# mit-han-lab/litepose

Hardware: AMD Instinct MI355X
Metric: images/sec end-to-end (backbone+deconv+AE-group), LitePose-XS@256 b64 (higher is better)
Workload: dtype f32

## Files before the change

### litepose_amd/csrc/ae_api.cpp

```cpp
#include <hip/hip_runtime.h>

#include <cstring>
#include <string>

#include "../../include/litepose_amd.h"
#include "kernels.h"

extern "C" void lp_set_error_(const char* msg);

namespace {
int fail(int code, const char* msg) {
    lp_set_error_(msg);
    return code;
}
size_t align256(size_t v) { return (v + 255) / 256 * 256; }

int to_params(const lp_parse_params* p, lp::ParseParams& q) {
    if (!p) return fail(LP_ERR_INVALID_ARG, "null params");
    if (p->num_joints < 1 || p->num_joints > 32) return fail(LP_ERR_UNSUPPORTED, "num_joints must be 1..32");
    if (p->max_num_people < 1 || p->max_num_people > 32)
        return fail(LP_ERR_UNSUPPORTED, "max_num_people must be 1..32");
    if (!(p->detection_threshold >= 0.0)) return fail(LP_ERR_INVALID_ARG, "detection_threshold must be >= 0");
    if (p->nms_kernel < 1 || (p->nms_kernel & 1) == 0) return fail(LP_ERR_INVALID_ARG, "nms_kernel must be odd");
    q.J = p->num_joints;
// ... 116 lines not shown
    lp::ScaleTable t;
    for (int s = 0; s < lp::MAX_SCALES; ++s) t.s[s] = {nullptr, 0, 0};
    for (int s = 0; s < S; ++s) {
        if (!scales[s].mid) return fail(LP_ERR_INVALID_ARG, "null mid");
        if (scales[s].h1 < 1 || scales[s].w1 < 1 || scales[s].h1 > 32767 || scales[s].w1 > 32767)
            return fail(LP_ERR_INVALID_ARG, "stage-1 sizes must be 1..32767");
        t.s[s] = {scales[s].mid, scales[s].h1, scales[s].w1};
    }
    if (!project2image && (Hf != scales[0].h1 || Wf != scales[0].w1))
        return fail(LP_ERR_INVALID_ARG, "without project2image (Hf, Wf) is the first scale's stage-1 size");
    if (T == 2 && ((uintptr_t)d_tag & 7)) return fail(LP_ERR_INVALID_ARG, "d_tag must be 8-byte aligned");
    if ((int64_t)N * 4 * J > 0x7fffffff) return fail(LP_ERR_UNSUPPORTED, "N * J too large");
    lp::launch_tta_merge_scales(t, S, first_unit, N, J, T, project2image ? 1 : 0, Hf, Wf, d_det, d_tag,
                                (hipStream_t)stream);
    if (hipGetLastError() != hipSuccess) return fail(LP_ERR_HIP, "tta_merge_scales launch failed");
    return LP_OK;
}

int lp_maps_accumulate(float* d_acc, const float* d_src, int64_t count, void* stream) {
    if (!d_acc || !d_src) return fail(LP_ERR_INVALID_ARG, "null argument");
    if (count < 0) return fail(LP_ERR_INVALID_ARG, "negative count");
    if (((uintptr_t)d_acc | (uintptr_t)d_src) & 15) return fail(LP_ERR_INVALID_ARG, "maps must be 16-byte aligned");
    if (count == 0) return LP_OK;
    lp::launch_maps_accumulate(d_acc, d_src, (long)count, (hipStream_t)stream);
    if (hipGetLastError() != hipSuccess) return fail(LP_ERR_HIP, "accumulate launch failed");
    return LP_OK;
}

int lp_peaks_topk(const float* d_det, const float* d_tag, int N, int J, int H, int W, int T,
                  const lp_parse_params* p, float* d_val_k, int32_t* d_ind_k, float* d_tag_k, void* stream) {
    lp::ParseParams q;
    int rc = to_params(p, q);
    if (rc) return rc;
    if (!d_det || !d_tag || !d_val_k || !d_ind_k || !d_tag_k) return fail(LP_ERR_INVALID_ARG, "null argument");
    if (J != q.J || T < 1 || T > 4 || N < 1 || H < 1 || W < 1) return fail(LP_ERR_INVALID_ARG, "bad dims");
    (void)lp::launch_peaks_topk(d_det, d_tag, N, J, H, W, T, q, d_val_k, d_ind_k, d_tag_k, (hipStream_t)stream);
    if (hipGetLastError() != hipSuccess) return fail(LP_ERR_HIP, "peaks_topk launch failed");
    return LP_OK;
}

int lp_group(const float* d_val_k, const int32_t* d_ind_k, const float* d_tag_k, int N, int W, int T,
             const lp_parse_params* p, int pcap, float* d_ans, int32_t* d_count, void* stream) {
    lp::ParseParams q;
    int rc = to_params(p, q);
    if (rc) return rc;
    if (!d_val_k || !d_ind_k || !d_tag_k || !d_ans || !d_count) return fail(LP_ERR_INVALID_ARG, "null argument");
    if (T < 1 || T > 4 || pcap < 1 || N < 1) return fail(LP_ERR_INVALID_ARG, "bad dims");
    lp::launch_group(d_val_k, d_ind_k, d_tag_k, N, W, T, q, pcap, d_ans, d_count, (hipStream_t)stream);
    if (hipGetLastError() != hipSuccess) return fail(LP_ERR_HIP, "group launch failed");
    return LP_OK;
}

size_t lp_refine_workspace_bytes(int N, int pcap) {
    return align256((size_t)N * pcap * 4 * sizeof(float)) + align256((size_t)N * pcap * sizeof(unsigned));
}

int lp_adjust_refine(const float* d_det, const float* d_tag, int N, int J, int H, int W, int T, int pcap,
                     int do_adjust, int do_refine, float* d_ans, const int32_t* d_count, float* d_scores,
                     void* ws, size_t ws_bytes, void* stream) {
    if (!d_det || !d_tag || !d_ans || !d_count || !d_scores || !ws)
        return fail(LP_ERR_INVALID_ARG, "null argument");
    if (T < 1 || T > 2) return fail(LP_ERR_UNSUPPORTED, "refine supports tag dimension 1 or 2");
    if (J < 1 || J > 32 || pcap < 1 || pcap > 1024) return fail(LP_ERR_UNSUPPORTED, "J 1..32, pcap 1..1024");
    if (ws_bytes < lp_refine_workspace_bytes(N, pcap)) return fail(LP_ERR_WORKSPACE, "refine workspace too small");
    float* prev = (float*)ws;
    unsigned* miss = (unsigned*)((char*)ws + align256((size_t)N * pcap * 4 * sizeof(float)));
    hipStream_t s = (hipStream_t)stream;
    lp::launch_adjust_scores(d_det, d_tag, N, J, H, W, T, pcap, do_adjust, d_ans, d_count, d_scores, prev,
                             miss, s);
    if (do_refine) lp::launch_refine(d_det, d_tag, N, J, H, W, T, pcap, d_ans, d_count, prev, miss, s);
    if (hipGetLastError() != hipSuccess) return fail(LP_ERR_HIP, "adjust/refine launch failed");
    return LP_OK;
}

size_t lp_parse_workspace_bytes(int N, int J, int M, int T, int pcap) {
    const size_t e = (size_t)N * J * M;
    return align256(e * sizeof(float)) + align256(e * sizeof(int)) + align256(e * T * sizeof(float)) +
           lp_refine_workspace_bytes(N, pcap);
}

int lp_parse(const float* d_det, const float* d_tag, int N, int J, int H, int W, int T,
             const lp_parse_params* p, int pcap, int do_adjust, int do_refine, float* d_ans,
             int32_t* d_count, float* d_scores, void* ws, size_t ws_bytes, void* stream) {
    if (!p || !ws) return fail(LP_ERR_INVALID_ARG, "null argument");
    const int M = p->max_num_people;
    if (ws_bytes < lp_parse_workspace_bytes(N, J, M, T, pcap))
        return fail(LP_ERR_WORKSPACE, "parse workspace too small");
    const size_t e = (size_t)N * J * M;
    char* c = (char*)ws;
    float* val_k = (float*)c;            c += align256(e * sizeof(float));
    int* ind_k = (int*)c;                c += align256(e * sizeof(int));
    float* tag_k = (float*)c;            c += align256(e * T * sizeof(float));
    int rc = lp_peaks_topk(d_det, d_tag, N, J, H, W, T, p, val_k, ind_k, tag_k, stream);
    if (rc) return rc;
    rc = lp_group(val_k, ind_k, tag_k, N, W, T, p, pcap, d_ans, d_count, stream);
    if (rc) return rc;
    return lp_adjust_refine(d_det, d_tag, N, J, H, W, T, pcap, do_adjust, do_refine, d_ans, d_count,
                            d_scores, c, lp_refine_workspace_bytes(N, pcap), stream);
}

int lp_parse_mid(const float* d_mid, int N, int J, int h1, int w1, int T, const lp_parse_params* p, int pcap,
                 int do_adjust, int do_refine, float* d_ans, int32_t* d_count, float* d_scores, void* ws,
                 size_t ws_bytes, void* stream) {
    lp::ParseParams q;
    int rc = to_params(p, q);
    if (rc) return rc;
    if (!d_mid || !d_ans || !d_count || !d_scores || !ws) return fail(LP_ERR_INVALID_ARG, "null argument");
    if (J != q.J || T < 1 || T > 2 || N < 1 || h1 < 1 || w1 < 1) return fail(LP_ERR_INVALID_ARG, "bad dims");
    if (pcap < 1 || pcap > 1024) return fail(LP_ERR_UNSUPPORTED, "pcap 1..1024");
    const int M = q.M;
    if (ws_bytes < lp_parse_workspace_bytes(N, J, M, T, pcap))
        return fail(LP_ERR_WORKSPACE, "parse workspace too small");
    const size_t e = (size_t)N * J * M;
    char* c = (char*)ws;
    float* val_k = (float*)c;            c += align256(e * sizeof(float));
    int* ind_k = (int*)c;                c += align256(e * sizeof(int));
    float* tag_k = (float*)c;            c += align256(e * T * sizeof(float));
    float* prev = (float*)c;
    unsigned* miss = (unsigned*)(c + align256((size_t)N * pcap * 4 * sizeof(float)));
    hipStream_t s = (hipStream_t)stream;
    if (!lp::launch_peaks_topk_walk(d_mid, N, J, h1, w1, T, q, val_k, ind_k, tag_k, s) &&
        !lp::launch_peaks_topk_mid(d_mid, N, J, h1, w1, T, q, val_k, ind_k, tag_k, s))
        return fail(LP_ERR_UNSUPPORTED, "lp_parse_mid: NMS radius 1..3, max_num_people <= 64, width <= 1024, "
                                        "TAG_PER_JOINT only (use lp_tta_project + lp_parse)");
    lp::launch_group(val_k, ind_k, tag_k, N, 2 * w1, T, q, pcap, d_ans, d_count, s);
    lp::launch_adjust_scores_mid(d_mid, N, J, h1, w1, T, pcap, do_adjust, d_ans, d_count, d_scores, prev, miss, s);
    if (do_refine && !lp::launch_refine_dm(nullptr, d_mid, N, J, h1, w1, T, pcap, d_ans, d_count, prev, miss, s))
        lp::launch_refine_mid(d_mid, N, J, h1, w1, T, pcap, d_ans, d_count, prev, miss, s);
    if (hipGetLastError() != hipSuccess) return fail(LP_ERR_HIP, "parse_mid launch failed");
    return LP_OK;
}

int lp_parse_dm(const float* d_det, const float* d_mid, int N, int J, int h1, int w1, int T,
                const lp_parse_params* p, int pcap, int do_adjust, int do_refine, float* d_ans, int32_t* d_count,
                float* d_scores, void* ws, size_t ws_bytes, void* stream) {
    lp::ParseParams q;
    int rc = to_params(p, q);
    if (rc) return rc;
    if (!d_det || !d_mid || !d_ans || !d_count || !d_scores || !ws) return fail(LP_ERR_INVALID_ARG, "null argument");
    if (J != q.J || T < 1 || T > 2 || N < 1 || h1 < 1 || w1 < 1) return fail(LP_ERR_INVALID_ARG, "bad dims");
    if (pcap < 1 || pcap > 1024) return fail(LP_ERR_UNSUPPORTED, "pcap 1..1024");
    const int M = q.M, H = 2 * h1, W = 2 * w1;
    if (ws_bytes < lp_parse_workspace_bytes(N, J, M, T, pcap))
        return fail(LP_ERR_WORKSPACE, "parse workspace too small");
    const size_t e = (size_t)N * J * M;
    char* c = (char*)ws;
    float* val_k = (float*)c;            c += align256(e * sizeof(float));
    int* ind_k = (int*)c;                c += align256(e * sizeof(int));
    float* tag_k = (float*)c;            c += align256(e * T * sizeof(float));
    float* prev = (float*)c;
    unsigned* miss = (unsigned*)(c + align256((size_t)N * pcap * 4 * sizeof(float)));
    hipStream_t s = (hipStream_t)stream;
    if (w1 > 1024 || !lp::launch_peaks_topk(d_det, nullptr, N, J, H, W, T, q, val_k, ind_k, tag_k, s, d_mid))
        return fail(LP_ERR_UNSUPPORTED, "lp_parse_dm: NMS radius 1..3, max_num_people <= 64, W % 4 == 0, w1 <= 1024, "
                                        "TAG_PER_JOINT only (use lp_tta_project + lp_parse)");
    lp::launch_group(val_k, ind_k, tag_k, N, W, T, q, pcap, d_ans, d_count, s);
    lp::launch_adjust_scores_mid(d_mid, N, J, h1, w1, T, pcap, do_adjust, d_ans, d_count, d_scores, prev, miss, s);
    if (do_refine && !lp::launch_refine_dm(d_det, d_mid, N, J, h1, w1, T, pcap, d_ans, d_count, prev, miss, s))
        return fail(LP_ERR_UNSUPPORTED, "lp_parse_dm: refine not supported for this shape (its gate and the one above "
                                        "have diverged); use lp_tta_project + lp_parse");
    if (hipGetLastError() != hipSuccess) return fail(LP_ERR_HIP, "parse_dm launch failed");
    return LP_OK;
}

int lp_warp_invert(const double* h_trans, double* h_minv) {
    if (!h_trans || !h_minv) return fail(LP_ERR_INVALID_ARG, "null argument");
    double M[6] = {h_trans[0], h_trans[1], h_trans[2], h_trans[3], h_trans[4], h_trans[5]};
    double D = M[0] * M[4] - M[1] * M[3];
    D = D != 0.0 ? 1.0 / D : 0.0;
    const double A11 = M[4] * D, A22 = M[0] * D;
    M[0] = A11; M[1] *= -D;
    M[3] *= -D; M[4] = A22;
    const double b1 = -M[0] * M[2] - M[1] * M[5];
    const double b2 = -M[3] * M[2] - M[4] * M[5];
    M[2] = b1; M[5] = b2;
    for (int i = 0; i < 6; ++i) h_minv[i] = M[i];
    return LP_OK;
}

int lp_preprocess(const uint8_t* d_image, int H, int W, const double* h_trans, int Hd, int Wd,
                  const float* h_mean, const float* h_std, uint8_t* d_resized_u8, float* d_tensor,
                  void* stream) {
    return lp_preprocess_batch(d_image, 1, H, W, h_trans, Hd, Wd, h_mean, h_std, d_resized_u8, d_tensor, stream);
}

int lp_preprocess_batch(const uint8_t* d_image, int N, int H, int W, const double* h_trans, int Hd, int Wd,
                        const float* h_mean, const float* h_std, uint8_t* d_resized_u8, float* d_tensor,
                        void* stream) {
    if (!d_image || !h_trans || !h_mean || !h_std) return fail(LP_ERR_INVALID_ARG, "null argument");
    if (N < 1 || N > 65535) return fail(LP_ERR_INVALID_ARG, "N must be 1..65535");
    if (!d_resized_u8 && !d_tensor) return fail(LP_ERR_INVALID_ARG, "no output requested");
    if (H < 1 || W < 1 || Hd < 1 || Wd < 1 || H > 32767 || W > 32767 || Hd > 32767 || Wd > 32767)
        return fail(LP_ERR_INVALID_ARG, "image sizes must be 1..32767");
    for (int c = 0; c < 3; ++c)
        if (!(h_std[c] > 0.f)) return fail(LP_ERR_INVALID_ARG, "std must be positive");
    double M[6];
    lp_warp_invert(h_trans, M);
    lp::launch_warp_affine_norm(d_image, H, W, Hd, Wd, M, h_mean, h_std, d_resized_u8, d_tensor,
                                (hipStream_t)stream, N);
    if (hipGetLastError() != hipSuccess) return fail(LP_ERR_HIP, "preprocess launch failed");
    return LP_OK;
}

int lp_preprocess_batch_v(const uint8_t* d_src, size_t src_bytes, const lp_warp_desc* d_desc, int N, int Hd, int Wd,
                          const float* h_mean, const float* h_std, uint8_t* d_resized_u8, float* d_tensor,
                          void* stream) {
    if (!d_src || !d_desc || !h_mean || !h_std) return fail(LP_ERR_INVALID_ARG, "null argument");
    if (N < 1 || N > 65535) return fail(LP_ERR_INVALID_ARG, "N must be 1..65535");
    if (!d_resized_u8 && !d_tensor) return fail(LP_ERR_INVALID_ARG, "no output requested");
    if (src_bytes < 1 || src_bytes > (size_t)INT64_MAX) return fail(LP_ERR_INVALID_ARG, "src_bytes must be 1..INT64_MAX");
    if (Hd < 1 || Wd < 1 || Hd > 32767 || Wd > 32767) return fail(LP_ERR_INVALID_ARG, "image sizes must be 1..32767");
// ... 66 lines not shown
```

### litepose_amd/csrc/ae_kernels.hip

```cpp
#include <cstdlib>
#include <type_traits>

#include "ae_common.h"
#include "kernels.h"

namespace lp {

__global__ __launch_bounds__(256) void tta_stage_kernel(
    const float* __restrict__ out0, const float* __restrict__ out1, const float* __restrict__ out0f,
    const float* __restrict__ out1f, int N, int J, int C0, int C1, int tag_off, int h0, int w0, int h1,
    int w1, FlipIndex flip_index, float* __restrict__ mid) {
    const long total = (long)N * J * h1 * w1;
    const long g = (long)blockIdx.x * blockDim.x + threadIdx.x;
    if (g >= total) return;
    const int x = (int)(g % w1);
    const int y = (int)((g / w1) % h1);
    const int j = (int)((g / ((long)w1 * h1)) % J);
    const int n = (int)(g / ((long)w1 * h1 * J));
    const long plane1 = (long)h1 * w1, plane0 = (long)h0 * w0;
    const Lerp ly = lerp_coord(y, h0, h1);
    float* m = mid + (long)n * 4 * J * plane1 + (long)j * plane1 + (long)y * w1 + x;
    {
        const Lerp lx = lerp_coord(x, w0, w1);
        const float* p0 = out0 + (long)n * C0 * plane0;
        const float up_h = bilerp(p0 + (long)j * plane0, w0, ly, lx);
        const float up_t = bilerp(p0 + (long)(tag_off + j) * plane0, w0, ly, lx);
        const float o1 = out1[((long)n * C1 + j) * plane1 + (long)y * w1 + x];
        m[0] = (up_h + o1) / 2.f;
        m[2 * J * plane1] = up_t;
    }
    if (out0f) {
        const int xs = w1 - 1 - x;
        const int fj = flip_index.v[j];
        const Lerp lx = lerp_coord(xs, w0, w1);
        const float* p0 = out0f + (long)n * C0 * plane0;
        const float up_h = bilerp(p0 + (long)fj * plane0, w0, ly, lx);
        const float up_t = bilerp(p0 + (long)(tag_off + fj) * plane0, w0, ly, lx);
        const float o1 = out1f[((long)n * C1 + fj) * plane1 + (long)y * w1 + xs];
        m[1 * J * plane1] = (up_h + o1) / 2.f;
        m[3 * J * plane1] = up_t;
    }
}

constexpr int P2_ROWS = 8, P2_COLS = 32;
constexpr int S2_LR = P2_ROWS / 2 + 2;

template <bool ADD, int CG>
__global__ __launch_bounds__(256) void tta_stage2x_kernel(
    const float* __restrict__ out0, const float* __restrict__ out1, const float* __restrict__ out0f,
    const float* __restrict__ out1f, int J, int C0, int C1, int tag_off, int h0, int w0,
    FlipIndex flip_index, float* __restrict__ mid, const float* __restrict__ add0, const float* __restrict__ add1,
    const float* __restrict__ add0f, const float* __restrict__ add1f) {
// ... 1530 lines not shown
        switch (nk) {
            case 1: LP_SCAN(1); break;
            case 2: LP_SCAN(2); break;
            case 3: LP_SCAN(3); break;
            case 4: LP_SCAN(4); break;
            case 5: LP_SCAN(5); break;
            case 6: LP_SCAN(6); break;
            case 7: LP_SCAN(7); break;
            default: LP_SCAN(8); break;
        }
#undef LP_SCAN
#pragma unroll
        for (int k = 0; k < RCH; ++k) {
            if (k >= nk) break;
            float v = bv[k];
            int i = bi[k];
#pragma unroll
            for (int o = 32; o >= 1; o >>= 1) {
                const float ov = __shfl_xor(v, o, 64);
                const int oi = __shfl_xor(i, o, 64);
                if (ov > v || (ov == v && oi < i)) { v = ov; i = oi; }
            }
            if (lane == 0) { red_v[wave][k] = v; red_i[wave][k] = i; }
        }
        __syncthreads();
        if (tid < nk) {
            float v = red_v[0][tid];
            int i = red_i[0][tid];
            for (int w = 1; w < RF_THREADS / 64; ++w) {
                const float ov = red_v[w][tid];
                const int oi = red_i[w][tid];
                if (ov > v || (ov == v && oi < i)) { v = ov; i = oi; }
            }
            const int y = i / W, x = i - y * W;
            const float val = dp[i];
            float fx = (float)x + 0.5f, fy = (float)y + 0.5f;
            if (dp[(long)y * W + min(x + 1, W - 1)] > dp[(long)y * W + max(x - 1, 0)]) fx += 0.25f;
            else fx -= 0.25f;
            if (dp[(long)min(y + 1, H - 1) * W + x] > dp[(long)max(0, y - 1) * W + x]) fy += 0.25f;
            else fy -= 0.25f;
            if (val > 0.f) {
                const int q = plist[base + tid];
                float* o = ans + (((long)n * pcap + q) * J + j) * D;
                o[0] = fx;
                o[1] = fy;
                o[2] = val;
            }
        }
        __syncthreads();
    }
}


template <int T, bool DETMID, int RFM_THREADS = 512>
__global__ __launch_bounds__(DETMID ? RFM_THREADS : RF_THREADS) void refine_dm_kernel(const float* __restrict__ det,
                                                               const float* __restrict__ mid, int J, int h1, int w1,
                                                               int pcap, float* __restrict__ ans,
                                                               const int* __restrict__ count,
                                                               const float* __restrict__ prev,
                                                               const unsigned* __restrict__ miss) {
    constexpr int NT = DETMID ? RFM_THREADS : RF_THREADS;
    __shared__ int plist[GKEYS];
    __shared__ int pn;
    __shared__ float red_v[NT / 64][RCH];
    __shared__ int red_i[NT / 64][RCH];
    const int j = blockIdx.x, n = blockIdx.y;
    const int tid = threadIdx.x, lane = tid & 63, wave = tid >> 6;
    const int D = 3 + T;
    const int H = 2 * h1, W = 2 * w1, plane1 = h1 * w1;
    const int P = min(max(count[n], 0), min(pcap, GKEYS));
    if (wave == 0) {
        int c = 0;
        for (int q0 = 0; q0 < P; q0 += 64) {
            const int q = q0 + lane;
            const bool m = q < P && ((miss[(long)n * pcap + q] >> j) & 1u);
            const u64 b = __ballot(m);
            if (m) plist[c + __popcll(b & ((1ull << lane) - 1ull))] = q;
            c += __popcll(b);
        }
        if (lane == 0) pn = c;
    }
    __syncthreads();
    const int np = pn;
    if (np == 0) return;
    const float* dp = DETMID ? nullptr : det + ((long)n * J + j) * H * W;
    const float* tpl[2] = {mid_plane(mid, n, 2, j, J, plane1), mid_plane(mid, n, T == 2 ? 3 : 2, j, J, plane1)};
    const float* hpl[2] = {mid_plane(mid, n, 0, j, J, plane1), mid_plane(mid, n, T == 2 ? 1 : 0, j, J, plane1)};
    auto det_px = [&](int yy, int xx) -> float {
        if constexpr (DETMID) return det_at(mid, n, j, J, h1, w1, T, yy, xx);
        else return dp[(long)yy * W + xx];
    };
    const int strips = max(1, NT / w1);
    const int rps = (h1 + strips - 1) / strips;
    const bool live = tid < w1 * strips;
    const int c = live ? tid % w1 : 0, sidx = live ? tid / w1 : 0;
    const int ia = min(sidx * rps, h1), ib = live ? min(h1, ia + rps) : ia;
    const int c0 = max(c - 1, 0), c2 = min(c + 1, w1 - 1);
    const float lx0[2] = {c == 0 ? 1.f : 0.25f, 0.75f}, lx1[2] = {c == 0 ? 0.f : 0.75f, 0.25f};
    constexpr int RCHX = (DETMID && RFM_THREADS == 1024) ? 4 : RCH;
    for (int base = 0; base < np; base += RCHX) {
        const int nk = min(RCHX, np - base);
        float pt[RCHX][2];
        float bv[RCHX];
        int bi[RCHX];
#pragma unroll
        for (int k = 0; k < RCHX; ++k) {
            const int q = __builtin_amdgcn_readfirstlane(plist[base + (k < nk ? k : 0)]);
            pt[k][0] = prev[((long)n * pcap + q) * GT + 0];
            pt[k][1] = prev[((long)n * pcap + q) * GT + 1];
            bv[k] = -INFINITY;
            bi[k] = 0;
        }
        auto scan = [&](auto nkc) {
            constexpr int NK = decltype(nkc)::value;
            float hrow[T][3][2];
            float hdet[DETMID ? T : 1][3][2];
            auto hload = [&](int row, int slot) {
                const int rr = min(max(row, 0), h1 - 1);
                const unsigned ro = (unsigned)(rr * w1);
#pragma unroll
                for (int m = 0; m < T; ++m) {
                    const float* rp = tpl[m];
                    const float t0 = rp[ro + (unsigned)c0], t1 = rp[ro + (unsigned)c], t2 = rp[ro + (unsigned)c2];
                    hrow[m][slot][0] = lx0[0] * t0 + lx1[0] * t1;
                    hrow[m][slot][1] = lx0[1] * t1 + lx1[1] * t2;
                }
                if constexpr (DETMID) {
#pragma unroll
                    for (int m = 0; m < T; ++m) {
                        const float* rp = hpl[m];
                        const float t0 = rp[ro + (unsigned)c0], t1 = rp[ro + (unsigned)c], t2 = rp[ro + (unsigned)c2];
                        hdet[m][slot][0] = lx0[0] * t0 + lx1[0] * t1;
                        hdet[m][slot][1] = lx0[1] * t1 + lx1[1] * t2;
                    }
                }
            };
            if (ia < ib) {
                hload(ia - 1, 0);
                hload(ia, 1);
            }
#pragma unroll(RFM_THREADS == 1024 ? 1 : 2)
            for (int i = ia; i < ib; ++i) {
                hload(i + 1, 2);
                const float ly0[2] = {i == 0 ? 1.f : 0.25f, 0.75f}, ly1[2] = {i == 0 ? 0.f : 0.75f, 0.25f};
                float dq[2][2];
                if constexpr (DETMID) {
#pragma unroll
                    for (int a = 0; a < 2; ++a)
#pragma unroll
                        for (int b = 0; b < 2; ++b) {
                            const float v0 = ly0[a] * hdet[0][a][b] + ly1[a] * hdet[0][a + 1][b];
                            if (T == 2) {
                                const float v1 = ly0[a] * hdet[T - 1][a][b] + ly1[a] * hdet[T - 1][a + 1][b];
                                dq[a][b] = (v0 + v1) / 2.0f;
                            } else {
                                dq[a][b] = v0;
                            }
                        }
                } else {
                    const float2 d0 = *reinterpret_cast<const float2*>(dp + (long)(2 * i) * W + 2 * c);
                    const float2 d1 = *reinterpret_cast<const float2*>(dp + (long)(2 * i + 1) * W + 2 * c);
                    dq[0][0] = d0.x; dq[0][1] = d0.y; dq[1][0] = d1.x; dq[1][1] = d1.y;
                }
#pragma unroll
                for (int a = 0; a < 2; ++a)
#pragma unroll
                    for (int b = 0; b < 2; ++b) {
                        const float t0 = ly0[a] * hrow[0][a][b] + ly1[a] * hrow[0][a + 1][b];
                        const float t1 = T == 2 ? ly0[a] * hrow[T - 1][a][b] + ly1[a] * hrow[T - 1][a + 1][b] : 0.f;
                        const int idx = (2 * i + a) * W + 2 * c + b;
#pragma unroll
                        for (int k = 0; k < NK; ++k) {
                            const float da = t0 - pt[k][0];
                            float s2 = da * da;
                            if (T == 2) {
                                const float db = t1 - pt[k][1];
                                s2 = s2 + db * db;
                            }
                            const float v = dq[a][b] - rint_sqrt(s2);
                            if (v > bv[k]) { bv[k] = v; bi[k] = idx; }
                        }
                    }
#pragma unroll
                for (int m = 0; m < T; ++m)
#pragma unroll
                    for (int b = 0; b < 2; ++b) {
                        hrow[m][0][b] = hrow[m][1][b];
                        hrow[m][1][b] = hrow[m][2][b];
                        if constexpr (DETMID) {
                            hdet[m][0][b] = hdet[m][1][b];
                            hdet[m][1][b] = hdet[m][2][b];
                        }
                    }
            }
        };
        if constexpr (RCHX <= 4) {
            switch (nk) {
                case 1: scan(std::integral_constant<int, 1>()); break;
                case 2: scan(std::integral_constant<int, 2>()); break;
                case 3: scan(std::integral_constant<int, 3>()); break;
                default: scan(std::integral_constant<int, RCHX>()); break;
            }
        } else {
            switch (nk) {
                case 1: scan(std::integral_constant<int, 1>()); break;
                case 2: scan(std::integral_constant<int, 2>()); break;
                case 3: scan(std::integral_constant<int, 3>()); break;
                case 4: scan(std::integral_constant<int, 4>()); break;
                case 5: scan(std::integral_constant<int, 5>()); break;
                case 6: scan(std::integral_constant<int, 6>()); break;
                case 7: scan(std::integral_constant<int, 7>()); break;
                default: scan(std::integral_constant<int, 8>()); break;
            }
        }
#pragma unroll
        for (int k = 0; k < RCHX; ++k) {
            if (k >= nk) break;
            float v = bv[k];
            int i = bi[k];
#pragma unroll
            for (int o = 32; o >= 1; o >>= 1) {
                const float ov = __shfl_xor(v, o, 64);
                const int oi = __shfl_xor(i, o, 64);
                if (ov > v || (ov == v && oi < i)) { v = ov; i = oi; }
            }
            if (lane == 0) { red_v[wave][k] = v; red_i[wave][k] = i; }
        }
        __syncthreads();
        if (tid < nk) {
            float v = red_v[0][tid];
            int i = red_i[0][tid];
            for (int w = 1; w < NT / 64; ++w) {
                const float ov = red_v[w][tid];
                const int oi = red_i[w][tid];
                if (ov > v || (ov == v && oi < i)) { v = ov; i = oi; }
            }
            const int y = i / W, x = i - y * W;
            const float val = det_px(y, x);
            float fx = (float)x + 0.5f, fy = (float)y + 0.5f;
            if (det_px(y, min(x + 1, W - 1)) > det_px(y, max(x - 1, 0))) fx += 0.25f;
            else fx -= 0.25f;
            if (det_px(min(y + 1, H - 1), x) > det_px(max(0, y - 1), x)) fy += 0.25f;
            else fy -= 0.25f;
            if (val > 0.f) {
                const int q = plist[base + tid];
                float* o = ans + (((long)n * pcap + q) * J + j) * D;
                o[0] = fx;
                o[1] = fy;
                o[2] = val;
            }
        }
        __syncthreads();
    }
}

bool launch_refine_dm(const float* det, const float* mid, int N, int J, int h1, int w1, int T, int pcap, float* ans,
                      const int* count, const float* prev, const unsigned* miss, hipStream_t s) {
    if (w1 > (det ? RF_THREADS : 512) || T < 1 || T > 2) return false;
#define LP_RD(TV, DM, NTV)                                                                                 \
    hipLaunchKernelGGL((refine_dm_kernel<TV, DM, NTV>), dim3(J, N), dim3(DM ? NTV : RF_THREADS), 0, s, det, mid, J, h1, w1, \
                       pcap, ans, count, prev, miss)
    const bool small = w1 <= 128;
    const bool few = !det && (long)N * J <= 256;
    if (T == 2) { if (det) LP_RD(2, false, 512); else if (small && !few) LP_RD(2, true, 256); else LP_RD(2, true, 512); }
    else { if (det) LP_RD(1, false, 512); else if (few) LP_RD(1, true, 1024); else if (small) LP_RD(1, true, 256); else LP_RD(1, true, 512); }
#undef LP_RD
    return true;
}

void launch_adjust_scores(const float* det, const float* tag, int N, int J, int H, int W, int T,
                          int pcap, int do_adjust, float* ans, const int* count, float* scores,
                          float* prev, unsigned* miss, hipStream_t s) {
    hipLaunchKernelGGL(adjust_scores_kernel, dim3(N), dim3(256), 0, s, det, tag, J, H, W, T, pcap,
                       do_adjust, ans, count, scores, prev, miss);
}

void launch_refine(const float* det, const float* tag, int N, int J, int H, int W, int T, int pcap,
                   float* ans, const int* count, const float* prev, const unsigned* miss,
                   hipStream_t s) {
    hipLaunchKernelGGL(refine_kernel, dim3(J, N), dim3(RF_THREADS), 0, s, det, tag, J, H, W, T, pcap, ans,
                       count, prev, miss);
}

__device__ __forceinline__ void final_preds_row(float* __restrict__ jt, double sx, double tx, double sy, double ty) {
    const double x = (double)jt[0], y = (double)jt[1];
    jt[0] = (float)(sx * x + tx);
    jt[1] = (float)(sy * y + ty);
}

__global__ void final_preds_kernel(float* __restrict__ ans, const int* __restrict__ count, int pcap,
                                   int J, int D, double sx, double tx, double sy, double ty) {
    const int n = blockIdx.x;
    const int P = min(max(count[n], 0), pcap);
    for (int e = threadIdx.x; e < P * J; e += blockDim.x)
        final_preds_row(ans + ((long)n * pcap * J + e) * D, sx, tx, sy, ty);
}

__global__ void final_preds_v_kernel(float* __restrict__ ans, const int* __restrict__ count, int pcap, int J, int D,
                                     const double* __restrict__ coef) {
    const int n = blockIdx.x;
    const int P = min(max(count[n], 0), pcap);
    const double sx = coef[4 * n], tx = coef[4 * n + 1], sy = coef[4 * n + 2], ty = coef[4 * n + 3];
    for (int e = threadIdx.x; e < P * J; e += blockDim.x)
        final_preds_row(ans + ((long)n * pcap * J + e) * D, sx, tx, sy, ty);
}

__device__ __forceinline__ int sat_int_rint(double v) {
    const double r = rint(v);
    return r >= 2147483647.0 ? 2147483647 : (r <= -2147483648.0 ? (int)-2147483648LL : (int)r);
}

__device__ __forceinline__ void warp_norm_pixel(const unsigned char* __restrict__ src, int H, int W, int Hd, int Wd,
                                                int x, int y, double m0, double m1, double m2, double m3, double m4,
                                                double m5, const float (&mean)[3], const float (&sd)[3],
                                                unsigned char* __restrict__ dst_u8, float* __restrict__ dst_f32) {
    const int adelta = sat_int_rint(m0 * (double)x * 1024.0), bdelta = sat_int_rint(m3 * (double)x * 1024.0);
    const int X0 = sat_int_rint((m1 * (double)y + m2) * 1024.0) + 16;
    const int Y0 = sat_int_rint((m4 * (double)y + m5) * 1024.0) + 16;
    const int X = (X0 + adelta) >> 5, Y = (Y0 + bdelta) >> 5;
// ... 89 lines not shown
```

### litepose_amd/csrc/ae_mid_kernels.hip

```cpp
#include <cstdlib>

#include "ae_common.h"
#include "kernels.h"

namespace lp {

constexpr int PM_THREADS = 1024;
constexpr int PM_BR = 32;
constexpr int PM_KPT = TOPK_CAP / PM_THREADS;

template <int R>
__global__ __launch_bounds__(PM_THREADS) void peaks_topk_mid_kernel(
    const float* __restrict__ mid, int J, int h1, int w1, int T, int M, float* __restrict__ val_k,
    int* __restrict__ ind_k, float* __restrict__ tag_k) {
    extern __shared__ __attribute__((aligned(16))) u64 list[];
    __shared__ u64 wmax[2][16];
    __shared__ int wcount[16];
    constexpr int WIN = 2 * R + 1, SEG = TOPK_CAP / 16;
    const int H = 2 * h1, W = 2 * w1, plane1 = h1 * w1;
    float* band = reinterpret_cast<float*>(list + TOPK_CAP);
    const int pl = blockIdx.x;
    const int j = pl % J, n = pl / J;
    const int tid = threadIdx.x, lane = tid & 63, wave = tid >> 6;
    const float* ph = mid_plane(mid, n, 0, j, J, plane1);
// ... 118 lines not shown
                __syncthreads();
                const int rows = min(PM_BR, H - yb);
                for (int idx = tid; idx < rows * W; idx += PM_THREADS) {
                    const int y = yb + idx / W, x = idx % W;
                    const float v = band_at(yb, y, x);
                    if (v > 0.f) {
                        const u64 k = ((u64)__float_as_uint(v) << 32) | (u64)(0xFFFFFFFFu - (unsigned)(y * W + x));
                        if (k < prev && k > best) {
                            bool peak = true;
                            for (int yy = max(y - R, 0); yy <= min(y + R, H - 1) && peak; ++yy)
                                for (int xx = max(x - R, 0); xx <= min(x + R, W - 1); ++xx)
                                    if (band_at(yb, yy, xx) > v) { peak = false; break; }
                            if (peak) best = k;
                        }
                    }
                }
            }
        }
        best = wave_max_u64(best);
        if (lane == 0) wmax[m & 1][wave] = best;
        __syncthreads();
        u64 bb = wmax[m & 1][0];
#pragma unroll
        for (int w = 1; w < 16; ++w) {
            const u64 t = wmax[m & 1][w];
            bb = t > bb ? t : bb;
        }
        if (tid == m) mine = bb;
        prev = bb;
        if (bb == 0ull) break;
    }
    if (tid < M) {
        const u64 k = mine;
        float v = 0.f;
        int idx = 0;
        if (k) {
            v = __uint_as_float((unsigned)(k >> 32));
            idx = (int)(0xFFFFFFFFu - (unsigned)(k & 0xFFFFFFFFull));
        }
        const long o = (long)pl * M + tid;
        val_k[o] = v;
        ind_k[o] = idx;
        const int Y = idx / W, X = idx - Y * W;
        for (int t = 0; t < T; ++t) tag_k[o * T + t] = k ? tag_at(mid, n, j, J, h1, w1, t, Y, X) : 0.f;
    }
}

__global__ __launch_bounds__(256) void adjust_scores_mid_kernel(const float* __restrict__ mid, int J, int h1,
                                                                int w1, int T, int pcap, int do_adjust,
                                                                float* __restrict__ ans,
                                                                const int* __restrict__ count,
                                                                float* __restrict__ scores,
                                                                float* __restrict__ prev,
                                                                unsigned* __restrict__ miss) {
    const int n = blockIdx.x;
    const int H = 2 * h1, W = 2 * w1;
    const int D = 3 + T;
    const int P = min(max(count[n], 0), pcap);
    float* a = ans + (long)n * pcap * J * D;
    if (do_adjust) {
        for (int e = threadIdx.x; e < P * J; e += blockDim.x) {
            float* jt = a + (long)e * D;
            if (jt[2] > 0.f) {
                const int j = e % J;
                float c0 = jt[0], c1 = jt[1];
                const int xi = (int)c0, yi = (int)c1;
                if (det_at(mid, n, j, J, h1, w1, T, yi, min(xi + 1, W - 1)) >
                    det_at(mid, n, j, J, h1, w1, T, yi, max(xi - 1, 0)))
                    c0 += 0.25f;
                else
                    c0 -= 0.25f;
                if (det_at(mid, n, j, J, h1, w1, T, min(yi + 1, H - 1), xi) >
                    det_at(mid, n, j, J, h1, w1, T, max(0, yi - 1), xi))
                    c1 += 0.25f;
                else
                    c1 -= 0.25f;
                jt[0] = c0 + 0.5f;
                jt[1] = c1 + 0.5f;
            }
        }
    }
    __syncthreads();
    for (int pidx = threadIdx.x; pidx < pcap; pidx += blockDim.x) {
        float sc = 0.f;
        unsigned mm = 0;
        float pv[GT] = {0.f, 0.f, 0.f, 0.f};
        if (pidx < P) {
            const float* pj = a + (long)pidx * J * D;
            if (J < 8) {
                float r = 0.f;
                for (int j = 0; j < J; ++j) r = r + pj[j * D + 2];
                sc = r / (float)J;
            } else {
                float r[8];
                for (int k = 0; k < 8; ++k) r[k] = pj[k * D + 2];
                int i = 8;
                for (; i < J - (J % 8); i += 8)
                    for (int k = 0; k < 8; ++k) r[k] = r[k] + pj[(i + k) * D + 2];
                float res = ((r[0] + r[1]) + (r[2] + r[3])) + ((r[4] + r[5]) + (r[6] + r[7]));
                for (; i < J; ++i) res = res + pj[i * D + 2];
                sc = res / (float)J;
            }
            int nd = 0;
            for (int j = 0; j < J; ++j) nd += pj[j * D + 2] > 0.f ? 1 : 0;
            const int q = nd / 4;
            for (int t = 0; t < T; ++t) {
                float part[4] = {0.f, 0.f, 0.f, 0.f};
                int k = 0;
                for (int j = 0; j < J; ++j) {
// ... 148 lines not shown
                const int oi = red_i[w][tid];
                if (ov > v || (ov == v && oi < i)) { v = ov; i = oi; }
            }
            if (i == 0x7fffffff) i = 0;
            const int y = i / W, x = i - y * W;
            const float val = det_at(mid, n, j, J, h1, w1, T, y, x);
            float fx = (float)x + 0.5f, fy = (float)y + 0.5f;
            if (det_at(mid, n, j, J, h1, w1, T, y, min(x + 1, W - 1)) > det_at(mid, n, j, J, h1, w1, T, y, max(x - 1, 0)))
                fx += 0.25f;
            else
                fx -= 0.25f;
            if (det_at(mid, n, j, J, h1, w1, T, min(y + 1, H - 1), x) > det_at(mid, n, j, J, h1, w1, T, max(0, y - 1), x))
                fy += 0.25f;
            else
                fy -= 0.25f;
            if (val > 0.f) {
                const int q = plist[base + tid];
                float* o = ans + (((long)n * pcap + q) * J + j) * D;
                o[0] = fx;
                o[1] = fy;
                o[2] = val;
            }
        }
        __syncthreads();
    }
}

bool launch_peaks_topk_mid(const float* mid, int N, int J, int h1, int w1, int T, const ParseParams& p,
                           float* val_k, int* ind_k, float* tag_k, hipStream_t s) {
    const int r = p.nms_k / 2, W = 2 * w1;
    if (r < 1 || r > 3 || p.M > 64 || W > PM_THREADS || T < 1 || T > 2 || !p.tag_per_joint) return false;
    const size_t lds = (size_t)TOPK_CAP * sizeof(u64) + (size_t)(PM_BR + 2 * r) * W * sizeof(float);
    if (lds > 150 * 1024) return false;
#define LP_PM(RV)                                                                                        \
    do {                                                                                                 \
        static size_t attr_##RV = 0;                                                                     \
        if (attr_##RV < lds) {                                                                           \
            (void)hipFuncSetAttribute(reinterpret_cast<const void*>(peaks_topk_mid_kernel<RV>),          \
                                      hipFuncAttributeMaxDynamicSharedMemorySize, (int)lds);             \
            attr_##RV = lds;                                                                             \
        }                                                                                                \
        hipLaunchKernelGGL((peaks_topk_mid_kernel<RV>), dim3(N * J), dim3(PM_THREADS), lds, s, mid, J, h1, w1, T, \
                           p.M, val_k, ind_k, tag_k);                                                    \
    } while (0)
    if (r == 2) LP_PM(2);
    else if (r == 1) LP_PM(1);
    else LP_PM(3);
#undef LP_PM
    return true;
}

void launch_adjust_scores_mid(const float* mid, int N, int J, int h1, int w1, int T, int pcap, int do_adjust,
                              float* ans, const int* count, float* scores, float* prev, unsigned* miss,
                              hipStream_t s) {
    hipLaunchKernelGGL(adjust_scores_mid_kernel, dim3(N), dim3(256), 0, s, mid, J, h1, w1, T, pcap, do_adjust, ans,
                       count, scores, prev, miss);
}

void launch_refine_mid(const float* mid, int N, int J, int h1, int w1, int T, int pcap, float* ans,
                       const int* count, const float* prev, const unsigned* miss, hipStream_t s) {
    const size_t lds = (size_t)4 * (RM_ROWS + 2) * (w1 + 2) * sizeof(float);
    static size_t attr = 0;
    if (attr < lds) {
        (void)hipFuncSetAttribute(reinterpret_cast<const void*>(refine_mid_kernel),
                                  hipFuncAttributeMaxDynamicSharedMemorySize, (int)lds);
        attr = lds;
    }
    hipLaunchKernelGGL(refine_mid_kernel, dim3(J, N), dim3(RM_THREADS), lds, s, mid, J, h1, w1, T, pcap, ans, count,
                       prev, miss);
}

}
```

### litepose_amd/csrc/kernels.h

```cpp
#pragma once
#include <hip/hip_runtime.h>
#include <stdint.h>

namespace lp {

enum Act { ACT_NONE = 0, ACT_RELU = 1, ACT_RELU6 = 2 };

bool uses_scratch(const void* kernel_fn);

extern thread_local const char* last_kernel_tag;

struct LaunchNote { int grid = 0, block = 0, lds = 0, wgs_per_cu = 0; };
extern thread_local LaunchNote last_launch;
extern thread_local bool launch_notes;
void note_launch(const void* fn, dim3 grid, dim3 block, size_t lds);
#define LP_LAUNCH(kern, grid, block, lds, stream, ...)                                                   \
    do {                                                                                                 \
        if (lp::launch_notes) lp::note_launch(reinterpret_cast<const void*>(kern), grid, block, lds);    \
        hipLaunchKernelGGL(kern, grid, block, lds, stream, __VA_ARGS__);                                 \
    } while (0)

#ifndef LP_NO_LDS_DMA
#define LP_STAGE_LOAD(reg, src, dst)                                                                  \
    __builtin_amdgcn_global_load_lds((const __attribute__((address_space(1))) void*)(src),           \
// ... 93 lines not shown
                hipStream_t s, bool f16 = false);
bool launch_pwb(const void* inA, int Ca, const void* inB, int Cb, const void* wf, const float* bias, const void* res,
                void* out, int N, int HW, int Cout, int act, bool out_f32, hipStream_t s, bool f16 = false);
bool launch_headb(const void* inA, int Ca, const void* inB, int Cb, const void* wtA, const float* wbA, const void* wtB,
                  const float* wbB, const void* wf, float* out, int N, int H, int W, int K, int Cout, hipStream_t s,
                  bool f16 = false);
bool launch_mbtb(const void* x, const void* w1, const float* b1f, const void* wrow, const void* w2, const float* b2f,
                 const void* res, void* out, int N, int Cin, int Cexp, int Cout, int H, int W, int K, int S,
                 hipStream_t s, int mode = 1, int mode_s2 = 1, int mode_q = 1, const void* wrow2 = nullptr, int mode_d = 1,
                 bool f16 = false);
int phase_trace_read(unsigned long long* host, int nwg);
int wg_trace_read(unsigned long long* host, int nwg, int sel);
bool launch_deconvb(const void* inA, int Ca, const void* inB, int Cb, const void* wf, const float* bias, void* out,
                    int N, int h, int w_, int Cout, hipStream_t s, bool f16 = false);
void launch_octet_to_planar(const void* in, float* out, int N, int C, int HW, hipStream_t s, bool f16 = false);

struct ParseParams {
    int J, M;
    double det_thr, tag_thr;
    int use_det_val, ignore_too_much, nms_k, tag_per_joint;
    int joint_order[32];
};

struct FlipIndex { int v[32]; };
bool launch_tta_stage(const float* out0, const float* out1, const float* out0f, const float* out1f,
                      int N, int J, int C0, int C1, int tag_off, int h0, int w0, int h1, int w1,
                      const FlipIndex& flip_index, float* mid, hipStream_t s, const float* add0 = nullptr,
                      const float* add1 = nullptr, const float* add0f = nullptr, const float* add1f = nullptr);
void launch_maps_accumulate(float* acc, const float* src, long count, hipStream_t s);
bool launch_tta_project(const float* mid, int N, int J, int h1, int w1, int Hp, int Wp, int T,
                        float* det, float* tag, hipStream_t s);
constexpr int MAX_SCALES = 8;
struct ScaleMid {
    const float* mid;
    int h1, w1;
};
static_assert(sizeof(ScaleMid) == 16, "ScaleMid must match lp_scale_mid (16 bytes)");
struct ScaleTable { ScaleMid s[MAX_SCALES]; };
void launch_tta_merge_scales(const ScaleTable& t, int S, int first_unit, int N, int J, int T, int project2image,
                             int Hf, int Wf, float* det, float* tag, hipStream_t s);

bool launch_peaks_topk(const float* det, const float* tag, int N, int J, int H, int W, int T,
                       const ParseParams& p, float* val_k, int* ind_k, float* tag_k, hipStream_t s,
                       const float* mid = nullptr);
void launch_group(const float* val_k, const int* ind_k, const float* tag_k, int N, int W, int T,
                  const ParseParams& p, int pcap, float* ans, int* count, hipStream_t s);
void launch_adjust_scores(const float* det, const float* tag, int N, int J, int H, int W, int T,
                          int pcap, int do_adjust, float* ans, const int* count, float* scores,
                          float* prev, unsigned* miss, hipStream_t s);
void launch_refine(const float* det, const float* tag, int N, int J, int H, int W, int T, int pcap,
                   float* ans, const int* count, const float* prev, const unsigned* miss,
                   hipStream_t s);
bool launch_refine_dm(const float* det, const float* mid, int N, int J, int h1, int w1, int T, int pcap, float* ans,
                      const int* count, const float* prev, const unsigned* miss, hipStream_t s);
bool launch_peaks_topk_walk(const float* mid, int N, int J, int h1, int w1, int T, const ParseParams& p,
                            float* val_k, int* ind_k, float* tag_k, hipStream_t s);
bool launch_peaks_topk_mid(const float* mid, int N, int J, int h1, int w1, int T, const ParseParams& p,
                           float* val_k, int* ind_k, float* tag_k, hipStream_t s);
void launch_adjust_scores_mid(const float* mid, int N, int J, int h1, int w1, int T, int pcap, int do_adjust,
                              float* ans, const int* count, float* scores, float* prev, unsigned* miss,
                              hipStream_t s);
void launch_refine_mid(const float* mid, int N, int J, int h1, int w1, int T, int pcap, float* ans,
                       const int* count, const float* prev, const unsigned* miss, hipStream_t s);
void launch_warp_affine_norm(const unsigned char* src, int H, int W, int Hd, int Wd, const double* minv,
                             const float* mean, const float* sd, unsigned char* dst_u8, float* dst_f32,
                             hipStream_t s, int nimg = 1);
void launch_final_preds(float* ans, const int* count, int N, int pcap, int J, int T,
                        double sx, double tx, double sy, double ty, hipStream_t s);
struct WarpDesc {
    long long src_offset;
    int H, W;
    double minv[6];
};
static_assert(sizeof(WarpDesc) == 64, "WarpDesc must match lp_warp_desc (64 bytes)");
void launch_warp_affine_norm_v(const unsigned char* src, long long src_bytes, const WarpDesc* desc, int N, int Hd,
                               int Wd, const float* mean, const float* sd, unsigned char* dst_u8, float* dst_f32,
                               hipStream_t s);
void launch_final_preds_v(float* ans, const int* count, int N, int pcap, int J, int T, const double* coef,
                          hipStream_t s);

void launch_fast_peaks(const float* det, const float* tmap, long tstride, int N, int J, int H, int W, float threshold,
                       int window, int M, int* count, float* val, float* tag, int* ind, hipStream_t s);
void launch_fast_assign(const int* count, const float* val, const float* tag, const int* ind, int N, int J, int M,
                        const int* joint_order, float tag_threshold, float* ans, int* num, hipStream_t s);

}
```

Before: 23110.

## Split refine scan into row strips with atomic-max merge and finish kernel

```diff
diff --git a/litepose_amd/csrc/ae_api.cpp b/litepose_amd/csrc/ae_api.cpp
--- a/litepose_amd/csrc/ae_api.cpp
+++ b/litepose_amd/csrc/ae_api.cpp
@@ -192,7 +192,8 @@
 }
 
 size_t lp_refine_workspace_bytes(int N, int pcap) {
-    return align256((size_t)N * pcap * 4 * sizeof(float)) + align256((size_t)N * pcap * sizeof(unsigned));
+    return align256((size_t)N * pcap * 4 * sizeof(float)) + align256((size_t)N * pcap * sizeof(unsigned)) +
+           (size_t)N * pcap * 32 * sizeof(unsigned long long);
 }
 
 int lp_adjust_refine(const float* d_det, const float* d_tag, int N, int J, int H, int W, int T, int pcap,
@@ -258,14 +259,15 @@
     float* tag_k = (float*)c;            c += align256(e * T * sizeof(float));
     float* prev = (float*)c;
     unsigned* miss = (unsigned*)(c + align256((size_t)N * pcap * 4 * sizeof(float)));
+    unsigned long long* slots = (unsigned long long*)((char*)miss + align256((size_t)N * pcap * sizeof(unsigned)));
     hipStream_t s = (hipStream_t)stream;
     if (!lp::launch_peaks_topk_walk(d_mid, N, J, h1, w1, T, q, val_k, ind_k, tag_k, s) &&
         !lp::launch_peaks_topk_mid(d_mid, N, J, h1, w1, T, q, val_k, ind_k, tag_k, s))
         return fail(LP_ERR_UNSUPPORTED, "lp_parse_mid: NMS radius 1..3, max_num_people <= 64, width <= 1024, "
                                         "TAG_PER_JOINT only (use lp_tta_project + lp_parse)");
     lp::launch_group(val_k, ind_k, tag_k, N, 2 * w1, T, q, pcap, d_ans, d_count, s);
-    lp::launch_adjust_scores_mid(d_mid, N, J, h1, w1, T, pcap, do_adjust, d_ans, d_count, d_scores, prev, miss, s);
-    if (do_refine && !lp::launch_refine_dm(nullptr, d_mid, N, J, h1, w1, T, pcap, d_ans, d_count, prev, miss, s))
+    lp::launch_adjust_scores_mid(d_mid, N, J, h1, w1, T, pcap, do_adjust, d_ans, d_count, d_scores, prev, miss, slots, s);
+    if (do_refine && !lp::launch_refine_dm(nullptr, d_mid, N, J, h1, w1, T, pcap, d_ans, d_count, prev, miss, slots, s))
         lp::launch_refine_mid(d_mid, N, J, h1, w1, T, pcap, d_ans, d_count, prev, miss, s);
     if (hipGetLastError() != hipSuccess) return fail(LP_ERR_HIP, "parse_mid launch failed");
     return LP_OK;
@@ -290,13 +292,14 @@
     float* tag_k = (float*)c;            c += align256(e * T * sizeof(float));
     float* prev = (float*)c;
     unsigned* miss = (unsigned*)(c + align256((size_t)N * pcap * 4 * sizeof(float)));
+    unsigned long long* slots = (unsigned long long*)((char*)miss + align256((size_t)N * pcap * sizeof(unsigned)));
     hipStream_t s = (hipStream_t)stream;
     if (w1 > 1024 || !lp::launch_peaks_topk(d_det, nullptr, N, J, H, W, T, q, val_k, ind_k, tag_k, s, d_mid))
         return fail(LP_ERR_UNSUPPORTED, "lp_parse_dm: NMS radius 1..3, max_num_people <= 64, W % 4 == 0, w1 <= 1024, "
                                         "TAG_PER_JOINT only (use lp_tta_project + lp_parse)");
     lp::launch_group(val_k, ind_k, tag_k, N, W, T, q, pcap, d_ans, d_count, s);
-    lp::launch_adjust_scores_mid(d_mid, N, J, h1, w1, T, pcap, do_adjust, d_ans, d_count, d_scores, prev, miss, s);
-    if (do_refine && !lp::launch_refine_dm(d_det, d_mid, N, J, h1, w1, T, pcap, d_ans, d_count, prev, miss, s))
+    lp::launch_adjust_scores_mid(d_mid, N, J, h1, w1, T, pcap, do_adjust, d_ans, d_count, d_scores, prev, miss, slots, s);
+    if (do_refine && !lp::launch_refine_dm(d_det, d_mid, N, J, h1, w1, T, pcap, d_ans, d_count, prev, miss, slots, s))
         return fail(LP_ERR_UNSUPPORTED, "lp_parse_dm: refine not supported for this shape (its gate and the one above "
                                         "have diverged); use lp_tta_project + lp_parse");
     if (hipGetLastError() != hipSuccess) return fail(LP_ERR_HIP, "parse_dm launch failed");
diff --git a/litepose_amd/csrc/ae_kernels.hip b/litepose_amd/csrc/ae_kernels.hip
--- a/litepose_amd/csrc/ae_kernels.hip
+++ b/litepose_amd/csrc/ae_kernels.hip
@@ -1,3 +1,4 @@
+#include <algorithm>
 #include <cstdlib>
 #include <type_traits>
 
@@ -1634,13 +1635,19 @@
 }
 
 
+__device__ __forceinline__ u64 refine_key(float v, int idx) {
+    const unsigned b = __float_as_uint(v == 0.f ? 0.f : v);
+    const unsigned o = (b & 0x80000000u) ? ~b : (b | 0x80000000u);
+    return ((u64)o << 32) | (u64)(0xFFFFFFFFu - (unsigned)idx);
+}
+
 template <int T, bool DETMID, int RFM_THREADS = 512>
 __global__ __launch_bounds__(DETMID ? RFM_THREADS : RF_THREADS) void refine_dm_kernel(const float* __restrict__ det,
                                                                const float* __restrict__ mid, int J, int h1, int w1,
-                                                               int pcap, float* __restrict__ ans,
-                                                               const int* __restrict__ count,
+                                                               int pcap, int R, const int* __restrict__ count,
                                                                const float* __restrict__ prev,
-                                                               const unsigned* __restrict__ miss) {
+                                                               const unsigned* __restrict__ miss,
+                                                               u64* __restrict__ slots) {
     constexpr int NT = DETMID ? RFM_THREADS : RF_THREADS;
     __shared__ int plist[GKEYS];
     __shared__ int pn;
@@ -1648,8 +1655,7 @@
     __shared__ int red_i[NT / 64][RCH];
     const int j = blockIdx.x, n = blockIdx.y;
     const int tid = threadIdx.x, lane = tid & 63, wave = tid >> 6;
-    const int D = 3 + T;
-    const int H = 2 * h1, W = 2 * w1, plane1 = h1 * w1;
+    const int W = 2 * w1, plane1 = h1 * w1;
     const int P = min(max(count[n], 0), min(pcap, GKEYS));
     if (wave == 0) {
         int c = 0;
@@ -1665,28 +1671,24 @@
     __syncthreads();
     const int np = pn;
     if (np == 0) return;
-    const float* dp = DETMID ? nullptr : det + ((long)n * J + j) * H * W;
+    const float* dp = DETMID ? nullptr : det + ((long)n * J + j) * (2 * h1) * W;
     const float* tpl[2] = {mid_plane(mid, n, 2, j, J, plane1), mid_plane(mid, n, T == 2 ? 3 : 2, j, J, plane1)};
     const float* hpl[2] = {mid_plane(mid, n, 0, j, J, plane1), mid_plane(mid, n, T == 2 ? 1 : 0, j, J, plane1)};
-    auto det_px = [&](int yy, int xx) -> float {
-        if constexpr (DETMID) return det_at(mid, n, j, J, h1, w1, T, yy, xx);
-        else return dp[(long)yy * W + xx];
-    };
+    const int r0 = min((int)blockIdx.z * R, h1), r1 = min(h1, r0 + R);
     const int strips = max(1, NT / w1);
-    const int rps = (h1 + strips - 1) / strips;
+    const int rps = (r1 - r0 + strips - 1) / strips;
     const bool live = tid < w1 * strips;
     const int c = live ? tid % w1 : 0, sidx = live ? tid / w1 : 0;
-    const int ia = min(sidx * rps, h1), ib = live ? min(h1, ia + rps) : ia;
+    const int ia = min(r0 + sidx * rps, r1), ib = live ? min(r1, ia + rps) : ia;
     const int c0 = max(c - 1, 0), c2 = min(c + 1, w1 - 1);
     const float lx0[2] = {c == 0 ? 1.f : 0.25f, 0.75f}, lx1[2] = {c == 0 ? 0.f : 0.75f, 0.25f};
-    constexpr int RCHX = (DETMID && RFM_THREADS == 1024) ? 4 : RCH;
-    for (int base = 0; base < np; base += RCHX) {
-        const int nk = min(RCHX, np - base);
-        float pt[RCHX][2];
-        float bv[RCHX];
-        int bi[RCHX];
-#pragma unroll
-        for (int k = 0; k < RCHX; ++k) {
+    for (int base = 0; base < np; base += RCH) {
+        const int nk = min(RCH, np - base);
+        float pt[RCH][2];
+        float bv[RCH];
+        int bi[RCH];
+#pragma unroll
+        for (int k = 0; k < RCH; ++k) {
             const int q = __builtin_amdgcn_readfirstlane(plist[base + (k < nk ? k : 0)]);
             pt[k][0] = prev[((long)n * pcap + q) * GT + 0];
             pt[k][1] = prev[((long)n * pcap + q) * GT + 1];
@@ -1721,7 +1723,7 @@
                 hload(ia - 1, 0);
                 hload(ia, 1);
             }
-#pragma unroll(RFM_THREADS == 1024 ? 1 : 2)
+#pragma unroll 2
             for (int i = ia; i < ib; ++i) {
                 hload(i + 1, 2);
                 const float ly0[2] = {i == 0 ? 1.f : 0.25f, 0.75f}, ly1[2] = {i == 0 ? 0.f : 0.75f, 0.25f};
@@ -1776,27 +1778,18 @@
                     }
             }
         };
-        if constexpr (RCHX <= 4) {
-            switch (nk) {
-                case 1: scan(std::integral_constant<int, 1>()); break;
-                case 2: scan(std::integral_constant<int, 2>()); break;
-                case 3: scan(std::integral_constant<int, 3>()); break;
-                default: scan(std::integral_constant<int, RCHX>()); break;
-            }
-        } else {
-            switch (nk) {
-                case 1: scan(std::integral_constant<int, 1>()); break;
-                case 2: scan(std::integral_constant<int, 2>()); break;
-                case 3: scan(std::integral_constant<int, 3>()); break;
-                case 4: scan(std::integral_constant<int, 4>()); break;
-                case 5: scan(std::integral_constant<int, 5>()); break;
-                case 6: scan(std::integral_constant<int, 6>()); break;
-                case 7: scan(std::integral_constant<int, 7>()); break;
-                default: scan(std::integral_constant<int, 8>()); break;
-            }
-        }
-#pragma unroll
-        for (int k = 0; k < RCHX; ++k) {
+        switch (nk) {
+            case 1: scan(std::integral_constant<int, 1>()); break;
+            case 2: scan(std::integral_constant<int, 2>()); break;
+            case 3: scan(std::integral_constant<int, 3>()); break;
+            case 4: scan(std::integral_constant<int, 4>()); break;
+            case 5: scan(std::integral_constant<int, 5>()); break;
+            case 6: scan(std::integral_constant<int, 6>()); break;
+            case 7: scan(std::integral_constant<int, 7>()); break;
+            default: scan(std::integral_constant<int, 8>()); break;
+        }
+#pragma unroll
+        for (int k = 0; k < RCH; ++k) {
             if (k >= nk) break;
             float v = bv[k];
             int i = bi[k];
@@ -1817,36 +1810,88 @@
                 const int oi = red_i[w][tid];
                 if (ov > v || (ov == v && oi < i)) { v = ov; i = oi; }
             }
-            const int y = i / W, x = i - y * W;
-            const float val = det_px(y, x);
-            float fx = (float)x + 0.5f, fy = (float)y + 0.5f;
-            if (det_px(y, min(x + 1, W - 1)) > det_px(y, max(x - 1, 0))) fx += 0.25f;
-            else fx -= 0.25f;
-            if (det_px(min(y + 1, H - 1), x) > det_px(max(0, y - 1), x)) fy += 0.25f;
-            else fy -= 0.25f;
-            if (val > 0.f) {
-                const int q = plist[base + tid];
-                float* o = ans + (((long)n * pcap + q) * J + j) * D;
-                o[0] = fx;
-                o[1] = fy;
-                o[2] = val;
-            }
+            const int q = plist[base + tid];
+            atomicMax(slots + ((long)n * pcap + q) * 32 + j, refine_key(v, i));
         }
         __syncthreads();
     }
 }
 
+template <bool DETMID>
+__global__ __launch_bounds__(256) void refine_finish_kernel(const float* __restrict__ det, const float* __restrict__ mid,
+                                                            int N, int J, int h1, int w1, int T, int pcap,
+                                                            float* __restrict__ ans, const int* __restrict__ count,
+                                                            const unsigned* __restrict__ miss,
+                                                            const u64* __restrict__ slots) {
+    const long e = (long)blockIdx.x * 256 + threadIdx.x;
+    if (e >= (long)N * pcap * J) return;
+    const int j = (int)(e % J), q = (int)((e / J) % pcap), n = (int)(e / ((long)J * pcap));
+    const int P = min(max(count[n], 0), min(pcap, GKEYS));
+    if (q >= P || !((miss[(long)n * pcap + q] >> j) & 1u)) return;
+    const u64 key = slots[((long)n * pcap + q) * 32 + j];
+    const int H = 2 * h1, W = 2 * w1, D = 3 + T;
+    const unsigned ui = 0xFFFFFFFFu - (unsigned)(key & 0xFFFFFFFFull);
+    if (key == 0 || ui >= (unsigned)(H * W)) return;
+    const int i = (int)ui;
+    const float* dp = DETMID ? nullptr : det + ((long)n * J + j) * H * W;
+    auto det_px = [&](int yy, int xx) -> float {
+        if constexpr (DETMID) return det_at(mid, n, j, J, h1, w1, T, yy, xx);
+        else return dp[(long)yy * W + xx];
+    };
+    const int y = i / W, x = i - y * W;
+    const float val = det_px(y, x);
+    float fx = (float)x + 0.5f, fy = (float)y + 0.5f;
+    if (det_px(y, min(x + 1, W - 1)) > det_px(y, max(x - 1, 0))) fx += 0.25f;
+    else fx -= 0.25f;
+    if (det_px(min(y + 1, H - 1), x) > det_px(max(0, y - 1), x)) fy += 0.25f;
+    else fy -= 0.25f;
+    if (val > 0.f) {
+        float* o = ans + (((long)n * pcap + q) * J + j) * D;
+        o[0] = fx;
+        o[1] = fy;
+        o[2] = val;
+    }
+}
+
+#ifndef LP_REFINE_CELLS
+#define LP_REFINE_CELLS 4096
+#endif
+#ifndef LP_REFINE_MIN_WGS
+#define LP_REFINE_MIN_WGS 512
+#endif
+constexpr int RF_MIN_ROWS = 4, RF_MIN_WGS = LP_REFINE_MIN_WGS;
+int refine_strip_rows(int N, int J, int h1, int w1) {
+    const long planes = (long)N * J;
+    int R = std::min(h1, std::max(RF_MIN_ROWS, LP_REFINE_CELLS / std::max(w1, 1)));
+    while (R > RF_MIN_ROWS && planes * ((h1 + R - 1) / R) < RF_MIN_WGS) R = std::max(RF_MIN_ROWS, (R + 1) / 2);
+    R = std::max(1, std::min(R, h1));
+    const int S = (h1 + R - 1) / R;
+    return (h1 + S - 1) / S;
+}
+int refine_strips(int N, int J, int h1, int w1) {
+    const int R = refine_strip_rows(N, J, h1, w1);
+    return (h1 + R - 1) / R;
+}
+
 bool launch_refine_dm(const float* det, const float* mid, int N, int J, int h1, int w1, int T, int pcap, float* ans,
-                      const int* count, const float* prev, const unsigned* miss, hipStream_t s) {
+                      const int* count, const float* prev, const unsigned* miss, u64* slots, hipStream_t s) {
     if (w1 > (det ? RF_THREADS : 512) || T < 1 || T > 2) return false;
+    const int R = refine_strip_rows(N, J, h1, w1), S = (h1 + R - 1) / R;
+    if (S > 65535) return false;
 #define LP_RD(TV, DM, NTV)                                                                                 \
-    hipLaunchKernelGGL((refine_dm_kernel<TV, DM, NTV>), dim3(J, N), dim3(DM ? NTV : RF_THREADS), 0, s, det, mid, J, h1, w1, \
-                       pcap, ans, count, prev, miss)
+    hipLaunchKernelGGL((refine_dm_kernel<TV, DM, NTV>), dim3(J, N, S), dim3(DM ? NTV : RF_THREADS), 0, s, det, mid, J, h1, \
+                       w1, pcap, R, count, prev, miss, slots)
     const bool small = w1 <= 128;
-    const bool few = !det && (long)N * J <= 256;
-    if (T == 2) { if (det) LP_RD(2, false, 512); else if (small && !few) LP_RD(2, true, 256); else LP_RD(2, true, 512); }
-    else { if (det) LP_RD(1, false, 512); else if (few) LP_RD(1, true, 1024); else if (small) LP_RD(1, true, 256); else LP_RD(1, true, 512); }
+    if (T == 2) { if (det) LP_RD(2, false, 512); else if (small) LP_RD(2, true, 256); else LP_RD(2, true, 512); }
+    else { if (det) LP_RD(1, false, 512); else if (small) LP_RD(1, true, 256); else LP_RD(1, true, 512); }
 #undef LP_RD
+    const long ne = (long)N * pcap * J;
+    if (det)
+        hipLaunchKernelGGL(refine_finish_kernel<false>, dim3((unsigned)((ne + 255) / 256)), dim3(256), 0, s, det, mid, N, J,
+                           h1, w1, T, pcap, ans, count, miss, slots);
+    else
+        hipLaunchKernelGGL(refine_finish_kernel<true>, dim3((unsigned)((ne + 255) / 256)), dim3(256), 0, s, det, mid, N, J,
+                           h1, w1, T, pcap, ans, count, miss, slots);
     return true;
 }
 
diff --git a/litepose_amd/csrc/ae_mid_kernels.hip b/litepose_amd/csrc/ae_mid_kernels.hip
--- a/litepose_amd/csrc/ae_mid_kernels.hip
+++ b/litepose_amd/csrc/ae_mid_kernels.hip
@@ -194,9 +194,11 @@
                                                                 const int* __restrict__ count,
                                                                 float* __restrict__ scores,
                                                                 float* __restrict__ prev,
-                                                                unsigned* __restrict__ miss) {
+                                                                unsigned* __restrict__ miss,
+                                                                u64* __restrict__ slots) {
     const int n = blockIdx.x;
     const int H = 2 * h1, W = 2 * w1;
+    for (int i = threadIdx.x; i < pcap * 32; i += blockDim.x) slots[(long)n * pcap * 32 + i] = 0ull;
     const int D = 3 + T;
     const int P = min(max(count[n], 0), pcap);
     float* a = ans + (long)n * pcap * J * D;
@@ -451,9 +453,9 @@
 
 void launch_adjust_scores_mid(const float* mid, int N, int J, int h1, int w1, int T, int pcap, int do_adjust,
                               float* ans, const int* count, float* scores, float* prev, unsigned* miss,
-                              hipStream_t s) {
+                              unsigned long long* slots, hipStream_t s) {
     hipLaunchKernelGGL(adjust_scores_mid_kernel, dim3(N), dim3(256), 0, s, mid, J, h1, w1, T, pcap, do_adjust, ans,
-                       count, scores, prev, miss);
+                       count, scores, prev, miss, slots);
 }
 
 void launch_refine_mid(const float* mid, int N, int J, int h1, int w1, int T, int pcap, float* ans,
diff --git a/litepose_amd/csrc/kernels.h b/litepose_amd/csrc/kernels.h
--- a/litepose_amd/csrc/kernels.h
+++ b/litepose_amd/csrc/kernels.h
@@ -169,14 +169,16 @@
                    float* ans, const int* count, const float* prev, const unsigned* miss,
                    hipStream_t s);
 bool launch_refine_dm(const float* det, const float* mid, int N, int J, int h1, int w1, int T, int pcap, float* ans,
-                      const int* count, const float* prev, const unsigned* miss, hipStream_t s);
+                      const int* count, const float* prev, const unsigned* miss, unsigned long long* slots, hipStream_t s);
+int refine_strip_rows(int N, int J, int h1, int w1);
+int refine_strips(int N, int J, int h1, int w1);
 bool launch_peaks_topk_walk(const float* mid, int N, int J, int h1, int w1, int T, const ParseParams& p,
                             float* val_k, int* ind_k, float* tag_k, hipStream_t s);
 bool launch_peaks_topk_mid(const float* mid, int N, int J, int h1, int w1, int T, const ParseParams& p,
                            float* val_k, int* ind_k, float* tag_k, hipStream_t s);
 void launch_adjust_scores_mid(const float* mid, int N, int J, int h1, int w1, int T, int pcap, int do_adjust,
                               float* ans, const int* count, float* scores, float* prev, unsigned* miss,
-                              hipStream_t s);
+                              unsigned long long* slots, hipStream_t s);
 void launch_refine_mid(const float* mid, int N, int J, int h1, int w1, int T, int pcap, float* ans,
                        const int* count, const float* prev, const unsigned* miss, hipStream_t s);
 void launch_warp_affine_norm(const unsigned char* src, int H, int W, int Hd, int Wd, const double* minv,
```

After: 23020. No clear change (-0.4%).
